# main--/rust-lz-fear

Measured on AMD Instinct MI355X. Metric: GiB/s compress + decompress, 4 MiB independent blocks, 1/2/4/8 MI355X, higher is better.
Workload: dtype u8

## Files before the change

rust-lz-fear_amd/build.py:

```python
import hashlib
import os
import subprocess
from concurrent.futures import ThreadPoolExecutor

PKG_DIR = os.path.dirname(os.path.abspath(__file__))
CSRC = os.path.join(PKG_DIR, "csrc")
ROOT = os.path.dirname(PKG_DIR)
LIB_PATH = os.environ.get("LZF_LIB_PATH") or os.path.join(PKG_DIR, "liblzfear_hip.so")
ANALYSIS_LIB_PATH = os.path.join(PKG_DIR, "liblzfear_hip_analysis.so")

PRODUCT_HIP = ["capi.hip", "capi_drivers.hip", "lz4_decompress_batched.hip", "lz4_decompress_paired.hip", "lz4_seg_front.hip", "lz4_seg_tiles.hip", "lz4_seg_order.hip", "lz4_seg_resolve.hip",
               "lz4_decompress_fed.hip", "lz4_decoded_size.hip", "lz4_decoded_size_seg.hip", "lz4_verify.hip", "lz4_compress.hip",
               "lz4_compress_compact.hip", "lz4_compress_team.hip", "aux_kernels.hip",
               "frame_device_scan.hip", "frame_device_decode.hip", "frame_device_index.hip", "frame_device_verify.hip", "frame_device_compress.hip"]
ANALYSIS_HIP = ["analysis/lz4_decompress.hip"]
CXX_SOURCES = ["frame.cpp", "host_staging.cpp", "capi_host.cpp"]
HEADERS = ["kernels.h", "lzf_device.h", "lz4_decompress_batch_phase.inc", "lz4_decompress_parse_phase.inc", "lz4_decompress_feed_phase.inc", "lzf_seg_common.h",
           "analysis/capi_analysis.inc", "capi_internal.h", "capi_order.h", "lzf_dispatch.h",
           "lzf_copy_helpers.h", "lzf_out_ring.h", "lzf_phase_timers.h", "lzf_parse_helpers.h", "lzf_compress_common.h", "lzf_simt.h", "lz4_compress_team.inc",
           "host_staging.h", "lzf_frame_scan.h", "lzf_stream_walk.h", "lzf_stream_index.h", "lzf_block_index.h", "frame_jobs.h", "frame_device_common.h", "lzf_frame_layout.h", "lzf_size_rules.h", "lzf_verify_rules.h", "lzf_chain_step.h", "lzf_history_trim.h", "lzf_fed_window.h", "frame_deliver_body.inc",
           os.path.join(ROOT, "include", "lzfear_hip.h"), os.path.join(ROOT, "include", "lzfear_frame.h")]


def _path(d):
    return d if os.path.isabs(d) else os.path.join(CSRC, d)


def hipcc():
    for c in ("/opt/rocm/bin/hipcc", "hipcc"):
        if os.path.isabs(c) and os.path.exists(c):
            return c
    return "hipcc"


def _sources(analysis):
    return PRODUCT_HIP + (ANALYSIS_HIP if analysis else []) + CXX_SOURCES


def _newest_header():
    return max((os.path.getmtime(_path(h)) for h in HEADERS if os.path.exists(_path(h))), default=0.0)


LAST_BUILD = {}


def build_library(force=False, verbose=False, defines=(), out=None, analysis=False):
    defines = list(defines)
    if (analysis or any(d.startswith("LZF_DBG") for d in defines)) and "LZF_ANALYSIS" not in defines:
        defines.append("LZF_ANALYSIS")
    analysis = "LZF_ANALYSIS" in defines
    extra = sorted(d for d in defines if d != "LZF_ANALYSIS")
    if out is None and extra:
        out = os.path.join(PKG_DIR, "liblzfear_hip_" + hashlib.sha1(" ".join(extra).encode()).hexdigest()[:10] + ".so")
    out = out or (ANALYSIS_LIB_PATH if analysis else LIB_PATH)
    srcs_t = max([os.path.getmtime(_path(s)) for s in _sources(analysis)] + [_newest_header()])
    if not force and os.path.exists(out) and os.path.getmtime(out) >= srcs_t:
        LAST_BUILD[out] = "reused (the library is newer than every source and header)"
        if verbose:
            print(f"[build] {os.path.basename(out)}: {LAST_BUILD[out]}", flush=True)
        return out
    tag = "product" if not defines else hashlib.sha1(" ".join(sorted(defines)).encode()).hexdigest()[:12]
    objdir = os.path.join(PKG_DIR, "_obj", tag)
    os.makedirs(objdir, exist_ok=True)
    hdr_t = _newest_header()
    base = [hipcc(), "--offload-arch=gfx950", "-O3", "-std=c++17", "-fPIC", "-I", os.path.join(ROOT, "include")] + [f"-D{d}" for d in defines]
    jobs = []
    for s in _sources(analysis):
        src = _path(s)
        obj = os.path.join(objdir, os.path.splitext(os.path.basename(s))[0] + ".o")
        stale = force or not os.path.exists(obj) or os.path.getmtime(obj) < max(os.path.getmtime(src), hdr_t)
        jobs.append((src, obj, stale))
    todo = [(s, o) for s, o, st in jobs if st]

    def compile_one(so):
        cmd = base + ["-c", so[0], "-o", so[1]]
        if verbose:
            print(" ".join(cmd), flush=True)
        subprocess.check_call(cmd)

    if todo:
        with ThreadPoolExecutor(max_workers=min(len(todo), int(os.environ.get("MAX_JOBS", 0)) or os.cpu_count() or 4)) as ex:
            list(ex.map(compile_one, todo))
    objs = [o for _, o, _ in jobs]
    if todo or not os.path.exists(out) or os.path.getmtime(out) < max(os.path.getmtime(o) for o in objs):
        cmd = [hipcc(), "--offload-arch=gfx950", "-shared", "-fPIC", "-o", out] + objs + ["-lpthread"]
        if verbose:
            print(" ".join(cmd), flush=True)
        subprocess.check_call(cmd)
    LAST_BUILD[out] = f"compiled {len(todo)} of {len(jobs)} sources with hipcc --offload-arch=gfx950, linked"
    if verbose:
        print(f"[build] {os.path.basename(out)}: {LAST_BUILD[out]}", flush=True)
    return out


DIST_LIB_PATH = os.path.join(PKG_DIR, "liblzfear_dist.so")


def build_dist_library(force=False, verbose=False):
    core = build_library(force=False, verbose=verbose)
    src = _path("dist_gather.hip")
    deps = [src, os.path.join(ROOT, "include", "lzfear_dist.h"), os.path.join(ROOT, "include", "lzfear_hip.h")]
    out = DIST_LIB_PATH
    if not force and os.path.exists(out) and os.path.getmtime(out) >= max(os.path.getmtime(d) for d in deps):
        LAST_BUILD[out] = "reused (the library is newer than every source and header)"
    else:
        cmd = [hipcc(), "--offload-arch=gfx950", "-O3", "-std=c++17", "-fPIC", "-shared", "-I", os.path.join(ROOT, "include"), "-o", out, src,
               "-L", os.path.dirname(core), "-l:" + os.path.basename(core), "-L", "/opt/rocm/lib", "-lrccl", "-Wl,-rpath,$ORIGIN", "-Wl,-rpath,/opt/rocm/lib"]
        if verbose:
            print(" ".join(cmd), flush=True)
        subprocess.check_call(cmd)
        LAST_BUILD[out] = "compiled dist_gather.hip with hipcc --offload-arch=gfx950, linked against librccl + liblzfear_hip"
    if verbose:
        print(f"[build] {os.path.basename(out)}: {LAST_BUILD[out]}", flush=True)
    return out


def build_analysis_library(force=False, verbose=False):
    return build_library(force=force, verbose=verbose, analysis=True)


COUNTER_BUILDS = (("LZF_DBG_ROUNDS=1", "LZF_DBG_FED_COUNT=0"), ("LZF_DBG_ROUNDS=2",))
FED_PERIODIC_COUNTER_BUILD = ("LZF_DBG_FED_COUNT=4",)
PARSE_TWIN_BUILD = ("LZF_ANALYSIS", "LZF_SEG_NOASM")


if __name__ == "__main__":
    import sys
    print(build_library(force="--force" in sys.argv, verbose=True, analysis="--analysis" in sys.argv))
```

rust-lz-fear_amd/csrc/lz4_seg_front.hip:

```cpp
#include "lzf_seg_common.h"
#include "lzf_dispatch.h"
#include <type_traits>

namespace lzf {
namespace {

constexpr uint32_t S = kSegRegion;
constexpr uint32_t kCB = kSegChunk;

__device__ __forceinline__ constexpr uint32_t seg_nch(uint32_t len) {
    return len <= kSegChunk ? 1u : 1u + (len - kSegChunk + kSegStride - 1u) / kSegStride;
}
static_assert(seg_nch(1u) == lzf_dispatch::seg_nch(1u) && seg_nch(kSegChunk) == lzf_dispatch::seg_nch(kSegChunk) && seg_nch(kSegChunk + 1u) == lzf_dispatch::seg_nch(kSegChunk + 1u) &&
              seg_nch(kSegChunk + kSegStride + 1u) == lzf_dispatch::seg_nch(kSegChunk + kSegStride + 1u) && seg_nch(lzf_dispatch::kSegMaxIn) == lzf_dispatch::seg_nch(lzf_dispatch::kSegMaxIn),
              "lzf_dispatch.h restates seg_nch");

}

__global__ __launch_bounds__(256) void lzf_seg_plan_kernel(seg_ctx c) {
    const uint32_t j = blockIdx.x * blockDim.x + threadIdx.x;
    if (j == 0u && c.rec_top) *c.rec_top = 0ull;
    if (j >= c.n_jobs) return;
    const lzf_decompress_job job = c.jobs[j];
    seg_job s;
    s.failed = 0; s.done = 0; s.ntok = 0; s.outb = 0; s.pad = 0; s.rec_off = 0; s.pad2 = 0;
    const bool in_window = job.input_len >= c.min_in && job.input_len <= c.max_in;
    if (c.size_only)
        s.eligible = (in_window && (job.input != nullptr || job.input_len == 0) && job.prefix_len < kMaxPosB && job.out_existing_len < kMaxPosB) ? 1u : 0u;
    else {
        const bool history = job.prefix_len < kMaxPosB && job.out_existing_len < kMaxPosB &&
                             (job.prefix_len == 0 || job.out_existing_len >= kSegPrefixReach || job.prefix != nullptr);
        s.eligible = ((c.fed || history) && in_window && job.input != nullptr && job.out != nullptr) ? 1u : 0u;
    }
    const uint32_t len = s.eligible ? (uint32_t)job.input_len : 0u;
    s.nch = s.eligible && !(c.size_only && len == 0u) ? seg_nch(len) : 0u;
    s.ntile = (len + kSegTile - 1u) / kSegTile;
    if (s.nch > c.maxch || s.ntile > c.maxtile) { s.eligible = 0; s.nch = 0; s.ntile = 0; }
    c.st[j] = s;
    if (c.est) {
        const uint32_t l31 = job.input_len > 0x7FFFFFFFull ? 0x7FFFFFFFu : (uint32_t)job.input_len;
        c.est[j] = (s.eligible ? 0u : l31 >> 4) + (c.len_shift < 32u ? l31 >> c.len_shift : 0u);
    }
}

#ifdef LZF_DBG_PARSE_TIME
__device__ unsigned long long lzf_dbg_parse_cycles[8];
#define PT_START() long long pt_t = clock64(); unsigned long long pt[4] = {0, 0, 0, 0}; uint32_t pt_n = 0, pt_hops[2] = {0, 0}
#define PT_MARK(i) do { const long long tn_ = clock64(); pt[i] += (unsigned long long)(tn_ - pt_t); pt_t = tn_; } while (0)
#define PT_CHUNK() (++pt_n)
#define PT_HOP_ASM "s_add_u32 %[nh], %[nh], 1\n\t"
#define PT_HOPS(mode, n) (pt_hops[mode] += (n))
#define PT_REPORT() do { if (lane == 0u && pt_n) { for (int i_ = 0; i_ < 4; ++i_) atomicAdd(&lzf_dbg_parse_cycles[i_], pt[i_]); \
                                                     atomicAdd(&lzf_dbg_parse_cycles[4], (unsigned long long)pt_n); atomicAdd(&lzf_dbg_parse_cycles[5], 1ull); \
                                                     atomicAdd(&lzf_dbg_parse_cycles[6], (unsigned long long)pt_hops[0]); atomicAdd(&lzf_dbg_parse_cycles[7], (unsigned long long)pt_hops[1]); } } while (0)
#else
#define PT_START() do { } while (0)
#define PT_MARK(i) do { } while (0)
#define PT_CHUNK() do { } while (0)
#define PT_HOP_ASM ""
#define PT_HOPS(mode, n) do { } while (0)
#define PT_REPORT() do { } while (0)
#endif
__global__ __launch_bounds__(64) void lzf_seg_parse_kernel(seg_ctx c) {
    __shared__ __attribute__((aligned(16))) uint8_t lds_parse[2u * 64u * 8u * 4u + kCB];
    static_assert(sizeof(lds_parse) == 20480, "eight chunks per CU: an eighth of 160 KiB each");
    uint32_t* const rowsA = reinterpret_cast<uint32_t*>(lds_parse);
    uint32_t* const rowsB = rowsA + 64u * 8u;
    const uint32_t j = seg_job_of(c, blockIdx.y);
    const seg_job sj = c.st[j];
    if (!sj.eligible) return;
    const uint32_t lane = threadIdx.x & 63u;
    const lzf_decompress_job job = c.jobs[j];
    cgu8* __restrict__ in = as_global(job.input);
    const uint32_t len = (uint32_t)job.input_len;
    uint8_t* const cbuf = lds_parse + 2u * 64u * 8u * 4u;
    const uint32_t cbuf_a = lds_addr(cbuf);
#define ROWA(w) rowsA[(w) * 64u + lane]
#define ROWB(w) rowsB[(w) * 64u + lane]

    PT_START();
    for (uint32_t h = blockIdx.x; h < sj.nch; h += gridDim.x) {
        const uint32_t cstart = h * kSegStride;
        __syncthreads();
        {
            const uint32_t avail = len - cstart < kCB ? len - cstart : kCB;
            cgu8* g = in + cstart;
            constexpr uint32_t kLd = kCB / 1024u;
            u32x4 v[kLd];
            if (avail >= 16u) {
#pragma unroll
                for (uint32_t k = 0; k < kLd; ++k) { const uint32_t i = k * 1024u + lane * 16u; v[k] = ld16(g + (i < avail - 16u ? i : avail - 16u)); }
            } else {
#pragma unroll
                for (uint32_t k = 0; k < kLd; ++k) v[k] = u32x4{0, 0, 0, 0};
            }
            if (avail == kCB) {
#pragma unroll
                for (uint32_t k = 0; k < kLd; ++k) *reinterpret_cast<u32x4*>(&cbuf[k * 1024u + lane * 16u]) = v[k];
            } else {
#pragma unroll
                for (uint32_t k = 0; k < kLd; ++k) { const uint32_t i = k * 1024u + lane * 16u; *reinterpret_cast<u32x4*>(&cbuf[i]) = i + 16u <= avail ? v[k] : u32x4{0, 0, 0, 0}; }
            }
            { const uint32_t t0 = avail & ~15u; if (t0 < kCB && lane < (avail & 15u)) cbuf[t0 + lane] = g[t0 + lane]; }
        }
        PT_MARK(0);
#pragma unroll
        for (uint32_t i = 0; i < 8u; ++i) { ROWA(i) = 0u; ROWB(i) = 0u; }
        const uint32_t room = len - cstart;
        const uint32_t fe = room > 24u ? (room - 24u < kCB - 2u ? room - 24u : kCB - 2u) : 0u;
        const uint32_t rb0 = lane * S, end_r = rb0 + S;

        auto rdb = [&](uint32_t q) -> uint32_t { const uint32_t r_ = q - cstart; if (r_ < kCB) return (uint32_t)cbuf[r_]; return (uint32_t)in[q]; };
        auto rd8 = [&](uint32_t q) -> uint64_t { const uint32_t r_ = q - cstart; if (r_ + 8u <= kCB) return lds_ld64u(cbuf_a + r_); return ld8(in + q); };
        auto token_next = [&](uint32_t p, uint32_t& next) -> bool { return token_next_gen(len, p, next, rd8, rdb); };
        auto walk = [&](uint32_t r, bool go, bool& merged, auto MODE) -> uint32_t {
            constexpr int mode = decltype(MODE)::value;
            const uint32_t stop = go ? (end_r < fe ? end_r : fe) : 0u;
            for (;;) {
#ifndef LZF_SEG_NOASM
                {
                    uint32_t mxp = 0x100u, q = r, mg = merged ? 1u : 0u;
                    const uint32_t stopv = stop;
                    const unsigned long long m0 = __ballot(go && !merged && r < stop);
                    uint32_t a_, w_, t_, x_, y_, bit_, mk_;
                    unsigned long long sv, sc, sb;
                    uint32_t nh = 0;
                    const uint32_t rowa2 = lds_addr(rowsA) + lane * 4u - (lane << 11), rowd = lds_addr(rowsB) - lds_addr(rowsA);
                    const uint32_t vzero = 0u, vff = 0xFFu, v100 = 0x100u, vffq = 0x100FFu, v100q = 0x10100u, vf00 = 0xF00u;
#define SEG_HOP_STEP_BACK(P, Q, L) \
                            "s_waitcnt lgkmcnt(0)\n\t" \
                            "v_cmp_ne_u32_sdwa vcc, %[w], %[mxp] src0_sel:BYTE_0 src1_sel:WORD_0\n\t"    \
                            "v_and_b32 %[a], 0xf00, %[w]\n\t" \
                            "v_bfe_u32 " L ", %[w], 12, 4\n\t" \
                            "v_cndmask_b32 %[t], -1, " P ", vcc\n\t"                                    \
                            "v_cndmask_b32 " P ", " Q ", " P ", vcc\n\t"
#define SEG_HOP_NEXT(P, Q, C100, VFF, L) \
                            "v_cmp_eq_u32_e64 %[sb], %[a], %[vf00]\n\t"                                 \
                            "v_cmp_eq_u32 vcc, 15, " L "\n\t"                                           \
                            "v_lshlrev_b32 %[bit], " P ", 1\n\t" \
                            "v_cndmask_b32_e64 %[mxp], " C100 ", " VFF ", %[sb]\n\t" \
                            "v_addc_co_u32 " Q ", %[sc], 3, " P ", %[sb]\n\t"                           \
                            "v_cmpx_lt_u32_e64 %[sc], %[t], %[stop]\n\t"
#define SEG_HOP_LITERALS(Q, L) \
                            "v_cndmask_b32_sdwa %[a], %[vz], %[w], vcc dst_sel:DWORD dst_unused:UNUSED_PAD src0_sel:DWORD src1_sel:BYTE_2\n\t" \
                            "v_addc_co_u32 " L ", vcc, " L ", %[a], vcc\n\t" \
                            "v_add_u32 " Q ", " Q ", " L "\n\t"
#define SEG_HOP_PARK(Q) \
                            "v_cmpx_ne_u32 vcc, 0xff, %[a]\n\t"                                         \
                            "v_cmpx_gt_u32 vcc, %[fe], " Q "\n\t"
#define SEG_HOP0(P, Q, C100, VFF) \
                            PT_HOP_ASM \
                            "v_add_u32 %[a], %[cbm1], " P "\n\t" \
                            "ds_read_b32 %[w], %[a]\n\t" \
                            SEG_HOP_STEP_BACK(P, Q, "%[x]") \
                            SEG_HOP_NEXT(P, Q, C100, VFF, "%[x]") \
                            SEG_HOP_LITERALS(Q, "%[x]") \
                            SEG_HOP_PARK(Q) \
                            "v_lshrrev_b32 %[x], 5, " P "\n\t" \
                            "v_lshl_add_u32 %[x], %[x], 8, %[rowa2]\n\t" \
                            "ds_or_b32 %[x], %[bit]\n\t"
#define SEG_HOP1(P, Q, C100, VFF) \
                            PT_HOP_ASM \
                            "v_add_u32 %[a], %[cbm1], " P "\n\t" \
                            "v_lshrrev_b32 %[x], 5, " P "\n\t" \
                            "ds_read_b32 %[w], %[a]\n\t" \
                            "v_lshl_add_u32 %[x], %[x], 8, %[rowa2]\n\t" \
                            "ds_read_b32 %[mk], %[x]\n\t" \
                            SEG_HOP_STEP_BACK(P, Q, "%[y]") \
                            "v_bfe_u32 %[mk], %[mk], " P ", 1\n\t" \
                            SEG_HOP_NEXT(P, Q, C100, VFF, "%[y]") \
                            "v_or_b32 %[mg], %[mg], %[mk]\n\t"                                          \
                            SEG_HOP_LITERALS(Q, "%[y]") \
                            "v_cmpx_eq_u32 vcc, 0, %[mk]\n\t" \
                            SEG_HOP_PARK(Q) \
                            "v_add_u32 %[x], %[x], %[rowd]\n\t"                                         \
                            "ds_or_b32 %[x], %[bit]\n\t"
                    if (mode == 0) {
                        asm volatile(
                            "s_mov_b64 %[sv], exec\n\t"
                            "s_and_b64 exec, exec, %[m0]\n\t"
                            "s_cbranch_execz Ld%=\n"
                            "Lw%=:\n\t"
                            SEG_HOP0("%[r]", "%[q]", "%[v100]", "%[vff]")
                            "s_cbranch_execz Ld%=\n\t"
                            SEG_HOP0("%[q]", "%[r]", "%[v100q]", "%[vffq]")
                            "s_cbranch_execnz Lw%=\n"
                            "Ld%=:\n\t"
                            "s_mov_b64 exec, %[sv]"
                            : [r] "+&v"(r), [q] "+&v"(q), [mxp] "+&v"(mxp),
                              [a] "=&v"(a_), [w] "=&v"(w_), [t] "=&v"(t_), [x] "=&v"(x_), [bit] "=&v"(bit_), [sv] "=&s"(sv), [sc] "=&s"(sc), [sb] "=&s"(sb), [nh] "+s"(nh)
                            : [cbm1] "s"(cbuf_a - 1u), [fe] "s"(fe), [stop] "v"(stopv), [rowa2] "v"(rowa2), [vz] "v"(vzero), [vff] "v"(vff), [v100] "v"(v100), [vffq] "v"(vffq), [v100q] "v"(v100q), [vf00] "v"(vf00), [m0] "s"(m0)
                            : "vcc", "scc", "memory");
                    } else {
                        asm volatile(
                            "s_mov_b64 %[sv], exec\n\t"
                            "s_and_b64 exec, exec, %[m0]\n\t"
                            "s_cbranch_execz Ld%=\n"
                            "Lw%=:\n\t"
                            SEG_HOP1("%[r]", "%[q]", "%[v100]", "%[vff]")
                            "s_cbranch_execz Ld%=\n\t"
                            SEG_HOP1("%[q]", "%[r]", "%[v100q]", "%[vffq]")
                            "s_cbranch_execnz Lw%=\n"
                            "Ld%=:\n\t"
                            "s_mov_b64 exec, %[sv]"
                            : [r] "+&v"(r), [q] "+&v"(q), [mxp] "+&v"(mxp), [mg] "+&v"(mg),
                              [a] "=&v"(a_), [w] "=&v"(w_), [t] "=&v"(t_), [x] "=&v"(x_), [y] "=&v"(y_), [bit] "=&v"(bit_), [mk] "=&v"(mk_), [sv] "=&s"(sv), [sc] "=&s"(sc), [sb] "=&s"(sb), [nh] "+s"(nh)
                            : [cbm1] "s"(cbuf_a - 1u), [fe] "s"(fe), [stop] "v"(stopv), [rowa2] "v"(rowa2), [rowd] "v"(rowd), [vz] "v"(vzero), [vff] "v"(vff), [v100] "v"(v100), [vffq] "v"(vffq), [v100q] "v"(v100q), [vf00] "v"(vf00), [m0] "s"(m0)
                            : "vcc", "scc", "memory");
                    }
#undef SEG_HOP_STEP_BACK
#undef SEG_HOP_NEXT
#undef SEG_HOP_LITERALS
#undef SEG_HOP_PARK
#undef SEG_HOP0
#undef SEG_HOP1
                    if (mxp & 0x10000u) r = q;
                    merged = mg != 0u;
                    PT_HOPS(mode, nh);
                }
#else
                uint32_t mxp = 0, q = r;
                bool act = go && !merged && r < stop, in_q = false;
                auto hop = [&](uint32_t& p, uint32_t& o, bool second) {
                    uint32_t lo;
                    asm volatile("ds_read_b32 %0, %1" : "=v"(lo) : "v"(cbuf_a + (act ? p : 0u) - 1u) : "memory");
                    uint32_t mk = 0;
                    const uint32_t bi = (act ? p : rb0) - rb0;
                    if (mode == 1) mk = *reinterpret_cast<const volatile uint32_t*>(&ROWA((bi >> 5) & 7u)) >> (bi & 31u);
                    asm volatile("s_waitcnt lgkmcnt(0)" ::: "memory");
                    const uint32_t e0 = lo & 255u;
                    if (act && mxp != 0u && e0 == 255u) { p = o; act = false; }
                    if (act) in_q = second;
                    if (act && p >= stop) act = false;
                    if (mode == 1) { if (act && (mk & 1u)) { merged = true; act = false; } }
                    if (act) {
                        const uint32_t L0 = (lo >> 12) & 15u, M0 = (lo >> 8) & 15u, b1 = (lo >> 16) & 255u;
                        const uint32_t isx = L0 == 15u ? 1u : 0u;
                        const uint32_t Lt = L0 + (isx ? b1 : 0u);
                        const uint32_t mx = M0 == 15u ? 1u : 0u;
                        const uint32_t pn = p + 3u + isx + Lt + mx;
                        const bool plain = !(isx && b1 == 255u) && pn < fe;
                        if (plain) {
                            if (mode == 0) ROWA((bi >> 5) & 7u) |= 1u << (bi & 31u); else ROWB((bi >> 5) & 7u) |= 1u << (bi & 31u);
                            o = pn; mxp = mx;
                        } else {
                            act = false;
                        }
                    }
                };
                while (__any(act)) {
                    hop(r, q, false);
                    if (!__any(act)) break;
                    hop(q, r, true);
                }
                if (in_q) r = q;
#endif
                const uint32_t pa = cstart + r;
                const bool slow = go && !merged && r < end_r && pa < len;
                if (!__any(slow)) break;
                if (slow) {
                    const uint32_t bi = r - rb0;
                    if (mode == 1 && ((ROWA((bi >> 5) & 7u) >> (bi & 31u)) & 1u)) merged = true;
                    else {
                        if (mode == 0) ROWA((bi >> 5) & 7u) |= 1u << (bi & 31u); else ROWB((bi >> 5) & 7u) |= 1u << (bi & 31u);
                        uint32_t nx;
                        if (!token_next(pa, nx)) nx = len;
                        r = nx - cstart;
                    }
                }
            }
            return r;
        };
        using M0T = std::integral_constant<int, 0>; using M1T = std::integral_constant<int, 1>;
        const bool in_input = cstart + rb0 < len;
        bool mdummy = false;
        const uint32_t x0 = walk(rb0, in_input, mdummy, M0T{});
        PT_MARK(1);
        uint32_t X = in_input ? x0 : 0u, walked = rb0, mpos = rb0;
        for (uint32_t pass = 0; pass < 80u; ++pass) {
            const uint32_t entry = wave_prev(wave_scan_max(X), 0u);
            const bool redo = in_input && entry != walked && lane != 0u;
            if (!__any(redo)) break;
            const bool inreg = redo && entry < end_r && cstart + entry < len;
            if (redo) {
                walked = entry;
#pragma unroll
                for (uint32_t i = 0; i < 8u; ++i) ROWB(i) = 0u;
            }
            bool mg = false;
            const uint32_t x1 = walk(inreg ? entry : end_r, inreg, mg, M1T{});
            if (redo) {
                if (!inreg) { X = entry; mpos = end_r; }
                else if (mg) { X = x0; mpos = x1; }
                else { X = x1; mpos = end_r; }
            }
        }
        PT_MARK(2);
        {
            const uint32_t mb = mpos - rb0;
            u32x4 o0, o1;
#pragma unroll
            for (uint32_t i = 0; i < 8u; ++i) {
                const uint32_t wb = mb >> 5;
                const uint32_t keep = i < wb ? 0u : i == wb ? ~((1u << (mb & 31u)) - 1u) : ~0u;
                const uint32_t v = in_input ? ((ROWA(i) & keep) | ROWB(i)) : 0u;
                if (i < 4u) o0[i] = v; else o1[i - 4u] = v;
            }
            LZF_GLOBAL u32x4* dst = (LZF_GLOBAL u32x4*)(c.bits + ((size_t)j * c.maxch + h) * kSegChunkWords + lane * 8u);
            dst[0] = o0; dst[1] = o1;
            if (!c.fed) {
                const uint32_t xm = __builtin_amdgcn_readlane(wave_scan_max(X), 63);
                uint64_t xe = (uint64_t)cstart + xm;
                if (xe > len) xe = len;
                if (lane == 0u) c.xexit[(size_t)j * c.maxch + h] = (uint32_t)xe;
            }
            if (c.est) {
                uint32_t cnt = 0;
                if (h == 0u || rb0 >= kSegOverlap) cnt = (uint32_t)(__popc(o0[0]) + __popc(o0[1]) + __popc(o0[2]) + __popc(o0[3]) + __popc(o1[0]) + __popc(o1[1]) + __popc(o1[2]) + __popc(o1[3]));
                const uint32_t tot = __builtin_amdgcn_readlane(wave_scan_add(cnt), 63);
                if (lane == 0u) __hip_atomic_fetch_add(&c.est[j], tot, __ATOMIC_RELAXED, __HIP_MEMORY_SCOPE_AGENT);
            }
        }
        PT_MARK(3);
        PT_CHUNK();
    }
    PT_REPORT();
}

#undef ROWA
#undef ROWB
#undef PT_START
#undef PT_MARK
#undef PT_CHUNK
#undef PT_HOP_ASM
#undef PT_HOPS
#undef PT_REPORT

__global__ __launch_bounds__(64) void lzf_seg_seam_kernel(seg_ctx c) {
    __shared__ uint16_t patch[kSegStride / 3u + 8u];
    constexpr uint32_t kWin = 2048;
    __shared__ __attribute__((aligned(16))) uint8_t wbytes[kWin + 128u];
    __shared__ uint32_t wbits[kWin / 32u + 2u];
    if (blockIdx.x >= c.g_n) return;
    const uint32_t j = c.grouped ? seg_job_of(c, blockIdx.x) : blockIdx.x;
    const seg_job sj = c.st[j];
    if (!sj.eligible) return;
    const uint32_t lane = threadIdx.x & 63u;
    const lzf_decompress_job job = c.jobs[j];
    cgu8* __restrict__ in = as_global(job.input);
    const uint32_t len = (uint32_t)job.input_len;
    LZF_GLOBAL uint32_t* const X = (LZF_GLOBAL uint32_t*)c.xexit + (size_t)j * c.maxch;
    LZF_GLOBAL uint32_t* const VF = (LZF_GLOBAL uint32_t*)c.vfrom + (size_t)j * c.maxch;
    LZF_GLOBAL uint32_t* const B = (LZF_GLOBAL uint32_t*)c.bits + (size_t)j * c.maxch * kSegChunkWords;
    auto bit = [&](uint32_t h, uint32_t pos) -> bool {
        const uint32_t r = pos - h * kSegStride;
        return (B[(size_t)h * kSegChunkWords + (r >> 5)] >> (r & 31u)) & 1u;
    };
    if (lane == 0u) VF[0] = 0u;
    bool carry_valid = false; uint32_t carry_e = 0;
    bool failed = false;
    for (uint32_t h0 = 1; h0 < sj.nch && !failed; h0 += 64u) {
        const uint32_t gn = sj.nch - h0 < 64u ? sj.nch - h0 : 64u;
        const uint32_t h = h0 + lane;
        const bool act = lane < gn;
        const uint32_t e = act ? X[h - 1u] : 0u;
        const uint32_t endh = h * kSegStride + kSegChunk;
        uint32_t code = 0;
        if (act) code = (e >= len || e >= endh) ? 1u : (bit(h, e) ? 0u : 2u);
        uint32_t k = 0;
        while (k < gn && !failed) {
            uint32_t e_true;
            if (!carry_valid) {
                const uint32_t kk0 = first_lane(__ballot(act && lane >= k && code != 0u));
                const uint32_t kk = kk0 < gn ? kk0 : gn;
                if (act && lane >= k && lane < kk) VF[h] = e;
                k = kk;
                if (k >= gn) break;
                e_true = __builtin_amdgcn_readlane(e, k);
            } else e_true = carry_e;
            const uint32_t hk = h0 + k;
            const uint32_t base = hk * kSegStride, endk = base + kSegChunk, ostart = base + kSegOverlap;
            if (e_true >= len || e_true >= endk) {
                if (lane == 0u) VF[hk] = kNone;
                carry_valid = true; carry_e = e_true;
            } else if (bit(hk, e_true)) {
                if (lane == 0u) VF[hk] = e_true;
                carry_valid = false;
            } else {
                uint32_t p = e_true, np = 0, mg = 0, err = 0;
                while (p < endk && p < len && !mg && !err) {
                    const uint32_t ws = p;
                    __syncthreads();
                    {
                        const uint32_t avail = len - ws < kWin + 128u ? len - ws : kWin + 128u;
                        for (uint32_t i = lane * 16u; i < kWin + 128u; i += 1024u) {
                            u32x4 v = u32x4{0, 0, 0, 0};
                            if (i + 16u <= avail) v = ld16(in + ws + i);
                            else if (i < avail) { for (uint32_t b = 0; i + b < avail; ++b) v[(b >> 2) & 3u] |= (uint32_t)in[ws + i + b] << ((b & 3u) * 8u); }
                            *reinterpret_cast<u32x4*>(&wbytes[i]) = v;
                        }
                        const uint32_t w0 = (ws - base) >> 5;
                        for (uint32_t i = lane; i < kWin / 32u + 2u; i += 64u)
                            wbits[i] = w0 + i < kSegChunkWords ? B[(size_t)hk * kSegChunkWords + w0 + i] : 0u;
                    }
                    __syncthreads();
                    if (lane == 0u) {
                        const uint32_t wb_a = lds_addr(wbytes);
                        auto rdb = [&](uint32_t q) -> uint32_t { const uint32_t r_ = q - ws; if (r_ < kWin + 128u) return (uint32_t)wbytes[r_]; return (uint32_t)in[q]; };
                        auto rd8 = [&](uint32_t q) -> uint64_t { const uint32_t r_ = q - ws; if (r_ + 8u <= kWin + 128u) return lds_ld64u(wb_a + r_); return ld8(in + q); };
                        const uint32_t bit0 = ((ws - base) >> 5) << 5;
                        while (p < endk && p < len && p - ws < kWin) {
                            const uint32_t rbit = p - base - bit0;
                            if (p != e_true && ((wbits[rbit >> 5] >> (rbit & 31u)) & 1u)) { mg = 1; break; }
                            patch[np++] = (uint16_t)(p - ostart);
                            uint32_t nx;
                            {
                                uint32_t w;
                                asm volatile("ds_read_b32 %0, %1\n\ts_waitcnt lgkmcnt(0)" : "=v"(w) : "v"(wb_a + (p - ws)) : "memory");
                                const uint32_t L0 = (w >> 4) & 15u, M0 = w & 15u, b1 = (w >> 8) & 255u;
                                const uint32_t q2 = p + 1u + (L0 == 15u ? 1u + 15u + b1 : L0);
                                if (!(L0 == 15u && b1 == 255u) && q2 + 3u <= len && q2 - ws + 3u <= kWin + 128u &&
                                    !(M0 == 15u && wbytes[q2 + 2u - ws] == 255u)) { p = q2 + 2u + (M0 == 15u ? 1u : 0u); continue; }
                            }
                            if (!token_next_gen(len, p, nx, rd8, rdb)) { err = 1; break; }
                            p = nx;
                        }
                    }
                    p = __builtin_amdgcn_readfirstlane(p); np = __builtin_amdgcn_readfirstlane(np);
                    mg = __builtin_amdgcn_readfirstlane(mg); err = __builtin_amdgcn_readfirstlane(err);
                }
                if (err) { failed = true; break; }
                uint32_t m = mg ? p : endk;
                {
                    const uint32_t w0 = kSegOverlap / 32u, mr = m - base;
                    for (uint32_t w = w0 + lane; w * 32u < mr; w += 64u) {
                        LZF_GLOBAL uint32_t* wp = &B[(size_t)hk * kSegChunkWords + w];
                        if (w * 32u + 32u <= mr) *wp = 0u;
                        else *wp &= ~((1u << (mr & 31u)) - 1u);
                    }
                    __threadfence();
                    for (uint32_t i = lane; i < np; i += 64u) {
                        const uint32_t r = (uint32_t)patch[i] + kSegOverlap;
                        atomicOr((uint32_t*)&B[(size_t)hk * kSegChunkWords + (r >> 5)], 1u << (r & 31u));
                    }
                    __threadfence();
                }
                if (lane == 0u) VF[hk] = ostart;
                if (mg) carry_valid = false; else { carry_valid = true; carry_e = p; }
            }
            ++k;
        }
    }
    if (failed && lane == 0u) c.st[j].failed = 1u;
}

}

#ifdef LZF_DBG_PARSE_TIME
extern "C" int lzf_debug_parse_timers(unsigned long long* out8, int reset) {
    if (out8 && hipMemcpyFromSymbol(out8, HIP_SYMBOL(lzf::lzf_dbg_parse_cycles), sizeof(unsigned long long) * 8u) != hipSuccess) return LZF_E_HIP;
    const unsigned long long z[8] = {0, 0, 0, 0, 0, 0, 0, 0};
    if (reset && hipMemcpyToSymbol(HIP_SYMBOL(lzf::lzf_dbg_parse_cycles), z, sizeof(z)) != hipSuccess) return LZF_E_HIP;
    return LZF_OK;
}
#endif
```

Measured before the change: 551.4.

## Replace pass-based seam re-walk with bounded-trip incremental parse scheduler

Replaces the up-to-80-pass loop in the segment parse kernel with an incremental scheduler. Previously each pass ran a full mode-1 walk to completion before propagating entry points across lanes. Now each lane advances at most K hop trips per round and publishes its exit as soon as it finishes, so restarts propagate without waiting for the slowest lane. The intent is to cut wave-wide idle time from divergent walk lengths. In exchange it adds more ballots, scans and state bookkeeping per round, and the scheduling logic is more complex.

Result: no change. 555.9 (median of 6 runs) (+0.8%).

```diff
diff --git a/rust-lz-fear_amd/build.py b/rust-lz-fear_amd/build.py
--- a/rust-lz-fear_amd/build.py
+++ b/rust-lz-fear_amd/build.py
@@ -18,7 +18,7 @@
 HEADERS = ["kernels.h", "lzf_device.h", "lz4_decompress_batch_phase.inc", "lz4_decompress_parse_phase.inc", "lz4_decompress_feed_phase.inc", "lzf_seg_common.h",
            "analysis/capi_analysis.inc", "capi_internal.h", "capi_order.h", "lzf_dispatch.h",
            "lzf_copy_helpers.h", "lzf_out_ring.h", "lzf_phase_timers.h", "lzf_parse_helpers.h", "lzf_compress_common.h", "lzf_simt.h", "lz4_compress_team.inc",
-           "host_staging.h", "lzf_frame_scan.h", "lzf_stream_walk.h", "lzf_stream_index.h", "lzf_block_index.h", "frame_jobs.h", "frame_device_common.h", "lzf_frame_layout.h", "lzf_size_rules.h", "lzf_verify_rules.h", "lzf_chain_step.h", "lzf_history_trim.h", "lzf_fed_window.h", "frame_deliver_body.inc",
+           "host_staging.h", "lzf_frame_scan.h", "lzf_stream_walk.h", "lzf_stream_index.h", "lzf_block_index.h", "frame_jobs.h", "frame_device_common.h", "lzf_frame_layout.h", "lzf_size_rules.h", "lzf_verify_rules.h", "lzf_chain_step.h", "lzf_history_trim.h", "lzf_fed_window.h", "lzf_parse_sched.h", "frame_deliver_body.inc",
            os.path.join(ROOT, "include", "lzfear_hip.h"), os.path.join(ROOT, "include", "lzfear_frame.h")]
 
 
diff --git a/rust-lz-fear_amd/csrc/lz4_seg_front.hip b/rust-lz-fear_amd/csrc/lz4_seg_front.hip
--- a/rust-lz-fear_amd/csrc/lz4_seg_front.hip
+++ b/rust-lz-fear_amd/csrc/lz4_seg_front.hip
@@ -1,11 +1,13 @@
 #include "lzf_seg_common.h"
 #include "lzf_dispatch.h"
+#include "lzf_parse_sched.h"
 #include <type_traits>
 
 namespace lzf {
 namespace {
 
 constexpr uint32_t S = kSegRegion;
+static_assert(kSegRegion == (uint32_t)kPschedRegion && kPschedTrips >= 1, "lzf_parse_sched.h restates the region; a boundary follows at least one trip");
 constexpr uint32_t kCB = kSegChunk;
 
 __device__ __forceinline__ constexpr uint32_t seg_nch(uint32_t len) {
@@ -44,21 +46,26 @@
 }
 
 #ifdef LZF_DBG_PARSE_TIME
-__device__ unsigned long long lzf_dbg_parse_cycles[8];
-#define PT_START() long long pt_t = clock64(); unsigned long long pt[4] = {0, 0, 0, 0}; uint32_t pt_n = 0, pt_hops[2] = {0, 0}
+__device__ unsigned long long lzf_dbg_parse_cycles[11];
+#define PT_START() long long pt_t = clock64(); unsigned long long pt[4] = {0, 0, 0, 0}; uint32_t pt_n = 0, pt_hops[2] = {0, 0}, pt_sched[3] = {0, 0, 0}
 #define PT_MARK(i) do { const long long tn_ = clock64(); pt[i] += (unsigned long long)(tn_ - pt_t); pt_t = tn_; } while (0)
 #define PT_CHUNK() (++pt_n)
 #define PT_HOP_ASM "s_add_u32 %[nh], %[nh], 1\n\t"
 #define PT_HOPS(mode, n) (pt_hops[mode] += (n))
+#define PT_BOUNDARY(scanned) (++pt_sched[(scanned) ? 1 : 0])
+#define PT_RESTARTS(mask) (pt_sched[2] += (uint32_t)__popcll(mask))
 #define PT_REPORT() do { if (lane == 0u && pt_n) { for (int i_ = 0; i_ < 4; ++i_) atomicAdd(&lzf_dbg_parse_cycles[i_], pt[i_]); \
                                                      atomicAdd(&lzf_dbg_parse_cycles[4], (unsigned long long)pt_n); atomicAdd(&lzf_dbg_parse_cycles[5], 1ull); \
-                                                     atomicAdd(&lzf_dbg_parse_cycles[6], (unsigned long long)pt_hops[0]); atomicAdd(&lzf_dbg_parse_cycles[7], (unsigned long long)pt_hops[1]); } } while (0)
+                                                     atomicAdd(&lzf_dbg_parse_cycles[6], (unsigned long long)pt_hops[0]); atomicAdd(&lzf_dbg_parse_cycles[7], (unsigned long long)pt_hops[1]); \
+                                                     for (int i_ = 0; i_ < 3; ++i_) atomicAdd(&lzf_dbg_parse_cycles[8 + i_], (unsigned long long)pt_sched[i_]); } } while (0)
 #else
 #define PT_START() do { } while (0)
 #define PT_MARK(i) do { } while (0)
 #define PT_CHUNK() do { } while (0)
 #define PT_HOP_ASM ""
 #define PT_HOPS(mode, n) do { } while (0)
+#define PT_BOUNDARY(scanned) do { } while (0)
+#define PT_RESTARTS(mask) do { } while (0)
 #define PT_REPORT() do { } while (0)
 #endif
 __global__ __launch_bounds__(64) void lzf_seg_parse_kernel(seg_ctx c) {
@@ -113,20 +120,61 @@
         auto rdb = [&](uint32_t q) -> uint32_t { const uint32_t r_ = q - cstart; if (r_ < kCB) return (uint32_t)cbuf[r_]; return (uint32_t)in[q]; };
         auto rd8 = [&](uint32_t q) -> uint64_t { const uint32_t r_ = q - cstart; if (r_ + 8u <= kCB) return lds_ld64u(cbuf_a + r_); return ld8(in + q); };
         auto token_next = [&](uint32_t p, uint32_t& next) -> bool { return token_next_gen(len, p, next, rd8, rdb); };
-        auto walk = [&](uint32_t r, bool go, bool& merged, auto MODE) -> uint32_t {
+        const uint32_t stop_r = end_r < fe ? end_r : fe;
+        auto general = [&](uint32_t& r, uint32_t& merged, auto MODE) {
             constexpr int mode = decltype(MODE)::value;
-            const uint32_t stop = go ? (end_r < fe ? end_r : fe) : 0u;
+            const uint32_t bi = r - rb0;
+            if (mode == 1 && ((ROWA((bi >> 5) & 7u) >> (bi & 31u)) & 1u)) { merged = 1u; return; }
+            if (mode == 0) ROWA((bi >> 5) & 7u) |= 1u << (bi & 31u); else ROWB((bi >> 5) & 7u) |= 1u << (bi & 31u);
+            uint32_t nx;
+            if (!token_next(cstart + r, nx)) nx = len;
+            r = nx - cstart;
+        };
+        using M0T = std::integral_constant<int, 0>; using M1T = std::integral_constant<int, 1>;
+#ifndef LZF_SEG_NOASM
+        const uint32_t rowa2 = lds_addr(rowsA) + lane * 4u - (lane << 11), rowd = lds_addr(rowsB) - lds_addr(rowsA);
+        const uint32_t vzero = 0u, vff = 0xFFu, v100 = 0x100u, vffq = 0x100FFu, v100q = 0x10100u, vf00 = 0xF00u;
+#else
+        auto hop_c = [&](uint32_t& p, uint32_t& o, uint32_t& mxp, bool& act, bool& in_q, uint32_t& merged, uint32_t stop, bool second, auto MODE) {
+            constexpr int mode = decltype(MODE)::value;
+            uint32_t lo;
+            asm volatile("ds_read_b32 %0, %1" : "=v"(lo) : "v"(cbuf_a + (act ? p : 0u) - 1u) : "memory");
+            uint32_t mk = 0;
+            const uint32_t bi = (act ? p : rb0) - rb0;
+            if (mode == 1) mk = *reinterpret_cast<const volatile uint32_t*>(&ROWA((bi >> 5) & 7u)) >> (bi & 31u);
+            asm volatile("s_waitcnt lgkmcnt(0)" ::: "memory");
+            const uint32_t e0 = lo & 255u;
+            if (act && e0 == (mxp & 0xFFFFu)) { p = o; act = false; }
+            if (act) in_q = second;
+            if (act && p >= stop) act = false;
+            if (mode == 1) { if (act && (mk & 1u)) { merged = 1u; act = false; } }
+            if (act) {
+                const uint32_t L0 = (lo >> 12) & 15u, M0 = (lo >> 8) & 15u, b1 = (lo >> 16) & 255u;
+                const uint32_t isx = L0 == 15u ? 1u : 0u;
+                const uint32_t Lt = L0 + (isx ? b1 : 0u);
+                const uint32_t mx = M0 == 15u ? 1u : 0u;
+                const uint32_t pn = p + 3u + isx + Lt + mx;
+                const bool plain = !(isx && b1 == 255u) && pn < fe;
+                if (plain) {
+                    if (mode == 0) ROWA((bi >> 5) & 7u) |= 1u << (bi & 31u); else ROWB((bi >> 5) & 7u) |= 1u << (bi & 31u);
+                    o = pn; mxp = mx ? 0xFFu : 0x100u;
+                } else {
+                    act = false;
+                }
+            }
+        };
+#endif
+        auto walk0 = [&](uint32_t r, bool go) -> uint32_t {
+            const uint32_t stop = go ? stop_r : 0u;
             for (;;) {
 #ifndef LZF_SEG_NOASM
                 {
-                    uint32_t mxp = 0x100u, q = r, mg = merged ? 1u : 0u;
+                    uint32_t mxp = 0x100u, q = r;
                     const uint32_t stopv = stop;
-                    const unsigned long long m0 = __ballot(go && !merged && r < stop);
-                    uint32_t a_, w_, t_, x_, y_, bit_, mk_;
+                    const unsigned long long m0 = __ballot(go && r < stop);
+                    uint32_t a_, w_, t_, x_, bit_;
                     unsigned long long sv, sc, sb;
                     uint32_t nh = 0;
-                    const uint32_t rowa2 = lds_addr(rowsA) + lane * 4u - (lane << 11), rowd = lds_addr(rowsB) - lds_addr(rowsA);
-                    const uint32_t vzero = 0u, vff = 0xFFu, v100 = 0x100u, vffq = 0x100FFu, v100q = 0x10100u, vf00 = 0xF00u;
 #define SEG_HOP_STEP_BACK(P, Q, L) \
                             "s_waitcnt lgkmcnt(0)\n\t" \
                             "v_cmp_ne_u32_sdwa vcc, %[w], %[mxp] src0_sel:BYTE_0 src1_sel:WORD_0\n\t"    \
@@ -175,126 +223,131 @@
                             SEG_HOP_PARK(Q) \
                             "v_add_u32 %[x], %[x], %[rowd]\n\t"                                         \
                             "ds_or_b32 %[x], %[bit]\n\t"
-                    if (mode == 0) {
-                        asm volatile(
-                            "s_mov_b64 %[sv], exec\n\t"
-                            "s_and_b64 exec, exec, %[m0]\n\t"
-                            "s_cbranch_execz Ld%=\n"
-                            "Lw%=:\n\t"
-                            SEG_HOP0("%[r]", "%[q]", "%[v100]", "%[vff]")
-                            "s_cbranch_execz Ld%=\n\t"
-                            SEG_HOP0("%[q]", "%[r]", "%[v100q]", "%[vffq]")
-                            "s_cbranch_execnz Lw%=\n"
-                            "Ld%=:\n\t"
-                            "s_mov_b64 exec, %[sv]"
-                            : [r] "+&v"(r), [q] "+&v"(q), [mxp] "+&v"(mxp),
-                              [a] "=&v"(a_), [w] "=&v"(w_), [t] "=&v"(t_), [x] "=&v"(x_), [bit] "=&v"(bit_), [sv] "=&s"(sv), [sc] "=&s"(sc), [sb] "=&s"(sb), [nh] "+s"(nh)
-                            : [cbm1] "s"(cbuf_a - 1u), [fe] "s"(fe), [stop] "v"(stopv), [rowa2] "v"(rowa2), [vz] "v"(vzero), [vff] "v"(vff), [v100] "v"(v100), [vffq] "v"(vffq), [v100q] "v"(v100q), [vf00] "v"(vf00), [m0] "s"(m0)
-                            : "vcc", "scc", "memory");
-                    } else {
-                        asm volatile(
-                            "s_mov_b64 %[sv], exec\n\t"
-                            "s_and_b64 exec, exec, %[m0]\n\t"
-                            "s_cbranch_execz Ld%=\n"
-                            "Lw%=:\n\t"
-                            SEG_HOP1("%[r]", "%[q]", "%[v100]", "%[vff]")
-                            "s_cbranch_execz Ld%=\n\t"
-                            SEG_HOP1("%[q]", "%[r]", "%[v100q]", "%[vffq]")
-                            "s_cbranch_execnz Lw%=\n"
-                            "Ld%=:\n\t"
-                            "s_mov_b64 exec, %[sv]"
-                            : [r] "+&v"(r), [q] "+&v"(q), [mxp] "+&v"(mxp), [mg] "+&v"(mg),
-                              [a] "=&v"(a_), [w] "=&v"(w_), [t] "=&v"(t_), [x] "=&v"(x_), [y] "=&v"(y_), [bit] "=&v"(bit_), [mk] "=&v"(mk_), [sv] "=&s"(sv), [sc] "=&s"(sc), [sb] "=&s"(sb), [nh] "+s"(nh)
-                            : [cbm1] "s"(cbuf_a - 1u), [fe] "s"(fe), [stop] "v"(stopv), [rowa2] "v"(rowa2), [rowd] "v"(rowd), [vz] "v"(vzero), [vff] "v"(vff), [v100] "v"(v100), [vffq] "v"(vffq), [v100q] "v"(v100q), [vf00] "v"(vf00), [m0] "s"(m0)
-                            : "vcc", "scc", "memory");
+                    asm volatile(
+                        "s_mov_b64 %[sv], exec\n\t"
+                        "s_and_b64 exec, exec, %[m0]\n\t"
+                        "s_cbranch_execz Ld%=\n"
+                        "Lw%=:\n\t"
+                        SEG_HOP0("%[r]", "%[q]", "%[v100]", "%[vff]")
+                        "s_cbranch_execz Ld%=\n\t"
+                        SEG_HOP0("%[q]", "%[r]", "%[v100q]", "%[vffq]")
+                        "s_cbranch_execnz Lw%=\n"
+                        "Ld%=:\n\t"
+                        "s_mov_b64 exec, %[sv]"
+                        : [r] "+&v"(r), [q] "+&v"(q), [mxp] "+&v"(mxp),
+                          [a] "=&v"(a_), [w] "=&v"(w_), [t] "=&v"(t_), [x] "=&v"(x_), [bit] "=&v"(bit_), [sv] "=&s"(sv), [sc] "=&s"(sc), [sb] "=&s"(sb), [nh] "+s"(nh)
+                        : [cbm1] "s"(cbuf_a - 1u), [fe] "s"(fe), [stop] "v"(stopv), [rowa2] "v"(rowa2), [vz] "v"(vzero), [vff] "v"(vff), [v100] "v"(v100), [vffq] "v"(vffq), [v100q] "v"(v100q), [vf00] "v"(vf00), [m0] "s"(m0)
+                        : "vcc", "scc", "memory");
+                    if (mxp & 0x10000u) r = q;
+                    PT_HOPS(0, nh);
+                }
+#else
+                uint32_t mxp = 0x100u, q = r;
+                bool act = go && r < stop, in_q = false;
+                uint32_t mdummy = 0u;
+                while (__any(act)) {
+                    hop_c(r, q, mxp, act, in_q, mdummy, stop, false, M0T{});
+                    if (!__any(act)) break;
+                    hop_c(q, r, mxp, act, in_q, mdummy, stop, true, M0T{});
+                }
+                if (in_q) r = q;
+#endif
+                const bool slow = go && r < end_r && cstart + r < len;
+                if (!__any(slow)) break;
+                uint32_t mdummy2 = 0u;
+                if (slow) general(r, mdummy2, M0T{});
+            }
+            return r;
+        };
+        const bool in_input = cstart + rb0 < len;
+        const uint32_t x0 = walk0(rb0, in_input);
+        PT_MARK(1);
+        lzf_psched_lane s;
+        lzf_psched_init(&s, rb0, x0, in_input);
+        bool dirty = true;
+        unsigned long long wkm = 0ull, lvm = 0ull, m0 = 0ull;
+        for (uint32_t nb = 0; nb < (uint32_t)kPschedCap; ++nb) {
+            const bool quiet = !dirty && wkm == lvm && lvm != 0ull;
+            PT_BOUNDARY(false);
+            if (quiet) m0 = lvm;
+            else {
+                const bool published = lzf_psched_publish(&s, x0, end_r, room) != 0;
+                if (dirty || __any(published)) {
+                    PT_BOUNDARY(true);
+                    const uint32_t entry = wave_prev(wave_scan_max(s.X), 0u);
+                    const uint32_t what = lzf_psched_restart(&s, entry, in_input, lane, end_r, room);
+                    if (what & LZF_PSCHED_RESTARTED) {
+#pragma unroll
+                        for (uint32_t i = 0; i < 8u; ++i) ROWB(i) = 0u;
                     }
+                    PT_RESTARTS(__ballot((what & LZF_PSCHED_WAS_WALKING) != 0u));
+                    dirty = __any((what & LZF_PSCHED_X_CHANGED) != 0u);
+                }
+                wkm = __ballot(s.walking != 0u);
+                if (lzf_psched_done(wkm != 0ull, dirty)) break;
+                if (!s.live) { s.q = s.r; s.mxp = 0x100u; }
+                m0 = __ballot(lzf_psched_hops(&s, stop_r) != 0);
+            }
+#ifndef LZF_SEG_NOASM
+            {
+                const uint32_t stopv = stop_r;
+                uint32_t a_, w_, t_, x_, y_, bit_, mk_;
+                unsigned long long sv, sc, sb;
+                uint32_t nh = 0, bud = (uint32_t)kPschedTrips - 1u;
+                asm volatile(
+                    "s_mov_b64 %[sv], exec\n\t"
+                    "s_and_b64 exec, exec, %[m0]\n\t"
+                    "s_cbranch_execz Ld%=\n"
+                    "Lw%=:\n\t"
+                    SEG_HOP1("%[r]", "%[q]", "%[v100]", "%[vff]")
+                    "s_cbranch_execz Ld%=\n\t"
+                    SEG_HOP1("%[q]", "%[r]", "%[v100q]", "%[vffq]")
+                    "s_cbranch_execz Ld%=\n\t"
+                    "s_sub_u32 %[bud], %[bud], 1\n\t"
+                    "s_cbranch_scc0 Lw%=\n"
+                    "Ld%=:\n\t"
+                    "s_mov_b64 %[lvm], exec\n\t"
+                    "s_mov_b64 exec, %[sv]\n\t"
+                    "v_cndmask_b32_e64 %[live], 0, 1, %[lvm]"
+                    : [r] "+&v"(s.r), [q] "+&v"(s.q), [mxp] "+&v"(s.mxp), [mg] "+&v"(s.merged), [bud] "+&s"(bud),
+                      [a] "=&v"(a_), [w] "=&v"(w_), [t] "=&v"(t_), [x] "=&v"(x_), [y] "=&v"(y_), [bit] "=&v"(bit_), [mk] "=&v"(mk_), [sv] "=&s"(sv), [sc] "=&s"(sc), [sb] "=&s"(sb), [live] "=&v"(s.live), [lvm] "=&s"(lvm), [nh] "+s"(nh)
+                    : [cbm1] "s"(cbuf_a - 1u), [fe] "s"(fe), [stop] "v"(stopv), [rowa2] "v"(rowa2), [rowd] "v"(rowd), [vz] "v"(vzero), [vff] "v"(vff), [v100] "v"(v100), [vffq] "v"(vffq), [v100q] "v"(v100q), [vf00] "v"(vf00), [m0] "s"(m0)
+                    : "vcc", "scc", "memory");
+                PT_HOPS(1, nh);
+            }
+#else
+            bool in_q = false;
+            {
+                bool act = (m0 >> lane) & 1ull;
+                uint32_t bud = (uint32_t)kPschedTrips;
+                while (__any(act)) {
+                    hop_c(s.r, s.q, s.mxp, act, in_q, s.merged, stop_r, false, M1T{});
+                    if (!__any(act)) break;
+                    hop_c(s.q, s.r, s.mxp, act, in_q, s.merged, stop_r, true, M1T{});
+                    if (!__any(act) || --bud == 0u) break;
+                }
+                s.live = act ? 1u : 0u;
+                lvm = __ballot(act);
+            }
+#endif
+            if (wkm != lvm) {
+#ifndef LZF_SEG_NOASM
+                if (!s.live && (s.mxp & 0x10000u)) s.r = s.q;
+#else
+                if (!s.live && in_q) s.r = s.q;
+#endif
+                if (lzf_psched_general(&s, end_r, room)) general(s.r, s.merged, M1T{});
+            }
+        }
+#ifndef LZF_SEG_NOASM
 #undef SEG_HOP_STEP_BACK
 #undef SEG_HOP_NEXT
 #undef SEG_HOP_LITERALS
 #undef SEG_HOP_PARK
 #undef SEG_HOP0
 #undef SEG_HOP1
-                    if (mxp & 0x10000u) r = q;
-                    merged = mg != 0u;
-                    PT_HOPS(mode, nh);
-                }
-#else
-                uint32_t mxp = 0, q = r;
-                bool act = go && !merged && r < stop, in_q = false;
-                auto hop = [&](uint32_t& p, uint32_t& o, bool second) {
-                    uint32_t lo;
-                    asm volatile("ds_read_b32 %0, %1" : "=v"(lo) : "v"(cbuf_a + (act ? p : 0u) - 1u) : "memory");
-                    uint32_t mk = 0;
-                    const uint32_t bi = (act ? p : rb0) - rb0;
-                    if (mode == 1) mk = *reinterpret_cast<const volatile uint32_t*>(&ROWA((bi >> 5) & 7u)) >> (bi & 31u);
-                    asm volatile("s_waitcnt lgkmcnt(0)" ::: "memory");
-                    const uint32_t e0 = lo & 255u;
-                    if (act && mxp != 0u && e0 == 255u) { p = o; act = false; }
-                    if (act) in_q = second;
-                    if (act && p >= stop) act = false;
-                    if (mode == 1) { if (act && (mk & 1u)) { merged = true; act = false; } }
-                    if (act) {
-                        const uint32_t L0 = (lo >> 12) & 15u, M0 = (lo >> 8) & 15u, b1 = (lo >> 16) & 255u;
-                        const uint32_t isx = L0 == 15u ? 1u : 0u;
-                        const uint32_t Lt = L0 + (isx ? b1 : 0u);
-                        const uint32_t mx = M0 == 15u ? 1u : 0u;
-                        const uint32_t pn = p + 3u + isx + Lt + mx;
-                        const bool plain = !(isx && b1 == 255u) && pn < fe;
-                        if (plain) {
-                            if (mode == 0) ROWA((bi >> 5) & 7u) |= 1u << (bi & 31u); else ROWB((bi >> 5) & 7u) |= 1u << (bi & 31u);
-                            o = pn; mxp = mx;
-                        } else {
-                            act = false;
-                        }
-                    }
-                };
-                while (__any(act)) {
-                    hop(r, q, false);
-                    if (!__any(act)) break;
-                    hop(q, r, true);
-                }
-                if (in_q) r = q;
-#endif
-                const uint32_t pa = cstart + r;
-                const bool slow = go && !merged && r < end_r && pa < len;
-                if (!__any(slow)) break;
-                if (slow) {
-                    const uint32_t bi = r - rb0;
-                    if (mode == 1 && ((ROWA((bi >> 5) & 7u) >> (bi & 31u)) & 1u)) merged = true;
-                    else {
-                        if (mode == 0) ROWA((bi >> 5) & 7u) |= 1u << (bi & 31u); else ROWB((bi >> 5) & 7u) |= 1u << (bi & 31u);
-                        uint32_t nx;
-                        if (!token_next(pa, nx)) nx = len;
-                        r = nx - cstart;
-                    }
-                }
-            }
-            return r;
-        };
-        using M0T = std::integral_constant<int, 0>; using M1T = std::integral_constant<int, 1>;
-        const bool in_input = cstart + rb0 < len;
-        bool mdummy = false;
-        const uint32_t x0 = walk(rb0, in_input, mdummy, M0T{});
-        PT_MARK(1);
-        uint32_t X = in_input ? x0 : 0u, walked = rb0, mpos = rb0;
-        for (uint32_t pass = 0; pass < 80u; ++pass) {
-            const uint32_t entry = wave_prev(wave_scan_max(X), 0u);
-            const bool redo = in_input && entry != walked && lane != 0u;
-            if (!__any(redo)) break;
-            const bool inreg = redo && entry < end_r && cstart + entry < len;
-            if (redo) {
-                walked = entry;
-#pragma unroll
-                for (uint32_t i = 0; i < 8u; ++i) ROWB(i) = 0u;
-            }
-            bool mg = false;
-            const uint32_t x1 = walk(inreg ? entry : end_r, inreg, mg, M1T{});
-            if (redo) {
-                if (!inreg) { X = entry; mpos = end_r; }
-                else if (mg) { X = x0; mpos = x1; }
-                else { X = x1; mpos = end_r; }
-            }
-        }
+#endif
+        const uint32_t X = s.X, mpos = s.mpos;
         PT_MARK(2);
         {
             const uint32_t mb = mpos - rb0;
@@ -334,6 +387,8 @@
 #undef PT_CHUNK
 #undef PT_HOP_ASM
 #undef PT_HOPS
+#undef PT_BOUNDARY
+#undef PT_RESTARTS
 #undef PT_REPORT
 
 __global__ __launch_bounds__(64) void lzf_seg_seam_kernel(seg_ctx c) {
@@ -459,8 +514,12 @@
 #ifdef LZF_DBG_PARSE_TIME
 extern "C" int lzf_debug_parse_timers(unsigned long long* out8, int reset) {
     if (out8 && hipMemcpyFromSymbol(out8, HIP_SYMBOL(lzf::lzf_dbg_parse_cycles), sizeof(unsigned long long) * 8u) != hipSuccess) return LZF_E_HIP;
-    const unsigned long long z[8] = {0, 0, 0, 0, 0, 0, 0, 0};
+    const unsigned long long z[11] = {0, 0, 0, 0, 0, 0, 0, 0, 0, 0, 0};
     if (reset && hipMemcpyToSymbol(HIP_SYMBOL(lzf::lzf_dbg_parse_cycles), z, sizeof(z)) != hipSuccess) return LZF_E_HIP;
     return LZF_OK;
 }
-#endif
+extern "C" int lzf_debug_parse_sched(unsigned long long* out3) {
+    if (hipMemcpyFromSymbol(out3, HIP_SYMBOL(lzf::lzf_dbg_parse_cycles), sizeof(unsigned long long) * 3u, sizeof(unsigned long long) * 8u) != hipSuccess) return LZF_E_HIP;
+    return LZF_OK;
+}
+#endif
diff --git a/rust-lz-fear_amd/csrc/lzf_parse_sched.h b/rust-lz-fear_amd/csrc/lzf_parse_sched.h
--- /dev/null
+++ b/rust-lz-fear_amd/csrc/lzf_parse_sched.h
@@ -0,0 +1,81 @@
+#ifndef LZF_PARSE_SCHED_H
+#define LZF_PARSE_SCHED_H
+
+#include <stdint.h>
+
+#if defined(__HIPCC__) || defined(__CUDACC__)
+#define LZF_PSCHED_HD __host__ __device__ static inline
+#else
+#define LZF_PSCHED_HD static inline
+#endif
+
+#ifndef LZF_PARSE_SCHED_K
+#define LZF_PARSE_SCHED_K 4
+#endif
+
+enum {
+    kPschedTrips = LZF_PARSE_SCHED_K,
+    kPschedRegion = 256,
+    kPschedCap = 64 * (kPschedRegion / 3 + 3),
+    LZF_PSCHED_RESTARTED = 1,
+    LZF_PSCHED_X_CHANGED = 2,
+    LZF_PSCHED_WAS_WALKING = 4
+};
+
+typedef struct {
+    uint32_t walking;
+    uint32_t live;
+    uint32_t r;
+    uint32_t q;
+    uint32_t mxp;
+    uint32_t merged;
+    uint32_t walked;
+    uint32_t X;
+    uint32_t mpos;
+} lzf_psched_lane;
+
+LZF_PSCHED_HD void lzf_psched_init(lzf_psched_lane* s, uint32_t rb0, uint32_t x0, int in_input) {
+    s->walking = 0u; s->live = 0u; s->r = rb0; s->q = rb0; s->mxp = 0x100u; s->merged = 0u;
+    s->walked = rb0; s->X = in_input ? x0 : 0u; s->mpos = rb0;
+}
+
+LZF_PSCHED_HD int lzf_psched_over(const lzf_psched_lane* s, uint32_t end_r, uint32_t room) {
+    return s->walking && !s->live && (s->merged || s->r >= end_r || s->r >= room);
+}
+
+LZF_PSCHED_HD int lzf_psched_publish(lzf_psched_lane* s, uint32_t x0, uint32_t end_r, uint32_t room) {
+    const int over = lzf_psched_over(s, end_r, room);
+    const uint32_t x = s->merged ? x0 : s->r;
+    const int changed = over && x != s->X;
+    s->mpos = over ? (s->merged ? s->r : end_r) : s->mpos;
+    s->X = over ? x : s->X;
+    s->walking = over ? 0u : s->walking;
+    return changed;
+}
+
+LZF_PSCHED_HD uint32_t lzf_psched_restart(lzf_psched_lane* s, uint32_t entry, int in_input, uint32_t lane, uint32_t end_r, uint32_t room) {
+    const int re = in_input && lane != 0u && entry != s->walked;
+    const int walk = re && entry < end_r && entry < room, jump = re && !walk;
+    const uint32_t what = (re ? (uint32_t)LZF_PSCHED_RESTARTED : 0u) | (re && s->walking ? (uint32_t)LZF_PSCHED_WAS_WALKING : 0u) |
+                          (jump && s->X != entry ? (uint32_t)LZF_PSCHED_X_CHANGED : 0u);
+    s->walked = re ? entry : s->walked;
+    s->live = re ? 0u : s->live; s->merged = re ? 0u : s->merged; s->mxp = re ? 0x100u : s->mxp;
+    s->r = walk ? entry : s->r; s->q = walk ? entry : s->q;
+    s->walking = re ? (walk ? 1u : 0u) : s->walking;
+    s->X = jump ? entry : s->X; s->mpos = jump ? end_r : s->mpos;
+    return what;
+}
+
+LZF_PSCHED_HD int lzf_psched_hops(const lzf_psched_lane* s, uint32_t stop) {
+    return s->walking && !s->merged && (s->live || s->r < stop);
+}
+
+LZF_PSCHED_HD int lzf_psched_general(const lzf_psched_lane* s, uint32_t end_r, uint32_t room) {
+    return s->walking && !s->live && !s->merged && s->r < end_r && s->r < room;
+}
+
+LZF_PSCHED_HD int lzf_psched_done(int any_walking, int dirty) {
+    return !any_walking && !dirty;
+}
+
+#endif
```
